# rsokolovskii/fl_scaling_sc_ldpc

Measured on AMD Instinct MI355X. Metric: MC codeword trials/sec, (4,8) SC-LDPC L=50 N=1000 eps=0.48 full BP, higher is better.
Workload: dtype u32

## Files before the change

fl_scaling_sc_ldpc_amd/csrc/sampler_v2.hip:

```cpp
#include "sampler_common.h"
#include "philox.h"

namespace {

using scldpc_dev::channel_erased;
using scldpc_dev::channel_tail;
using scldpc_dev::channel_undope;
using scldpc_dev::clear_hist_words;
using scldpc_dev::load_hist_words;
using scldpc_dev::store_hist_words;
using scldpc_dev::philox4x32_10;
using scldpc_dev::philox_prefix;
using scldpc_dev::philox_tail;
using scldpc_dev::philox_uniform;
using scldpc_dev::PhiloxPrefix;
using scldpc_dev::PhiloxUniform;
using scldpc_dev::wave_inclusive_scan;

constexpr int kThreads = scldpc::kSamplerThreads;
constexpr int kWaves = kThreads / 64;
using scldpc::kMaxDoped;
using scldpc::kWorkCap;

__device__ __forceinline__ uint32_t lds_add_rtn(uint32_t *p, uint32_t v)
{
    const uint32_t addr = (uint32_t)(uintptr_t)(__attribute__((address_space(3))) uint32_t *)p;
    uint32_t old;
    asm volatile("ds_add_rtn_u32 %0, %1, %2\n\ts_waitcnt lgkmcnt(0)" : "=v"(old) : "v"(addr), "v"(v) : "memory");
    return old;
}

struct S2Args {
    int L, cns_pos, vns_pos, n, S, D, nb, nw;
    int ntrials;
    int force_exact;
    int ndoped;
    int doped[kMaxDoped];
    uint32_t seed_lo, seed_hi;
    unsigned long long trial0;
    uint32_t thresh;
    int off_gpk, off_fix, off_stage, off_wsum;
    uint16_t *vn_adj16;
    uint16_t *cn_adj16;
    uint32_t *chan;
};

template <int ROWS, int CNMODE>
struct V2Layout {
    static constexpr int nb = ROWS * kThreads;
    static constexpr int off_gpk = nb, off_fix = off_gpk + nb, off_stage = off_fix + nb / 2;
    static constexpr int off_wsum = off_stage + (CNMODE != 0 ? nb / 2 : 0);
};

template <int KMAX, int ROWS, int CNMODE, bool PERSIST = false>
__global__ __launch_bounds__(kThreads, KMAX == 1 ? 8 : 4) __attribute__((amdgpu_num_sgpr(72))) void sample_philox_v2_kernel(const S2Args a)
{
    constexpr int DV = 4, DC_SHIFT = 3, E = 4 * KMAX;
    constexpr int LG = ROWS == 1 ? 10 : ROWS == 2 ? 11 : ROWS == 4 ? 12 : 13;
    constexpr int KSHIFT = 32 - LG - 2;
    constexpr bool INCL = KMAX == 1;
    static_assert(ROWS * kThreads == (1 << LG) && (INCL ? ROWS <= 4 : ROWS == 8), "ROWS is 1, 2, 4 (KMAX 1) or 8 (KMAX 2)");
    extern __shared__ uint32_t lds[];
    using Lay = V2Layout<ROWS, CNMODE>;
    const int off_gpk = INCL ? Lay::off_gpk : a.off_gpk, off_fix = INCL ? Lay::off_fix : a.off_fix;
    const int off_stage = INCL ? Lay::off_stage : a.off_stage, off_wsum = INCL ? Lay::off_wsum : a.off_wsum;
    uint32_t *hist = lds;
    uint32_t *gpk = lds + off_gpk;
    uint16_t *fix = reinterpret_cast<uint16_t *>(lds + off_fix);
    uint16_t *stage = reinterpret_cast<uint16_t *>(lds + off_stage);
    uint32_t *wsum = lds + off_wsum;
    uint32_t *wl = wsum + 32;

    const int tid = threadIdx.x, lane = tid & 63, wave = __builtin_amdgcn_readfirstlane(tid >> 6);
    const int S = a.S, nb = INCL ? ROWS * kThreads : a.nb;
    const int ncalls = S >> 2;
    bool own[KMAX];
#pragma unroll
    for (int k = 0; k < KMAX; k++) own[k] = tid + k * kThreads < ncalls;
    auto sock = [&](int e) { return (uint32_t)((tid + (e >> 2) * kThreads) * 4 + (e & 3)); };
    auto stage_entry = [&](int p, uint32_t sck) -> uint16_t {
        const int u = (int)(sck & 3u), t = (int)(sck >> 2);
        if ((unsigned)(p - u) >= (unsigned)a.L) return (uint16_t)0xFFFFu;
        return CNMODE == 1 ? (uint16_t)((p - u) * a.vns_pos + t) : (uint16_t)sck;
    };

    STAMP_DECL
    for (int b = tid; b < nb; b += kThreads) hist[b] = 0;
    if (tid == 0) { wsum[kWaves] = 0; wsum[kWaves + 1] = 0; }
    __syncthreads();
    auto sample_trial = [&](const int tr) {
    const unsigned long long trial = a.trial0 + (unsigned long long)tr;
    const uint32_t t_lo = (uint32_t)trial, t_hi = (uint32_t)(trial >> 32);
    uint32_t rowP[KMAX], rowQ[KMAX], rowR[KMAX];
#pragma unroll
    for (int k = 0; k < KMAX; k++) rowP[k] = rowQ[k] = rowR[k] = 0;
    PhiloxPrefix pre[KMAX];
#pragma unroll
    for (int k = 0; k < KMAX; k++) pre[k] = philox_prefix((uint32_t)(tid + k * kThreads), t_lo, t_hi, a.seed_lo, a.seed_hi);
    uint32_t nxt[E];
    {
        const PhiloxUniform un = philox_uniform(0u, t_lo, a.seed_lo, a.seed_hi);
#pragma unroll
        for (int k = 0; k < KMAX; k++) {
            uint32_t r[4] = {0, 0, 0, 0};
            if (own[k]) philox_tail(pre[k], un, a.seed_lo, a.seed_hi, r);
#pragma unroll
            for (int u = 0; u < 4; u++) nxt[4 * k + u] = r[u];
        }
    }
    for (int p = 0; p < a.D; p++) {
        STAMP(0);
        uint32_t key[E], slot[E], crowded = 0;
        auto word_of = [](uint32_t k) { return (k >> KSHIFT) & ~3u; };
        auto nib_of = [](uint32_t k) { return (k >> (KSHIFT - 2)) & 12u; };
#pragma unroll
        for (int e = 0; e < E; e++) {
            key[e] = nxt[e];
            const uint32_t sh = nib_of(key[e]);
            uint32_t *w = reinterpret_cast<uint32_t *>(reinterpret_cast<char *>(hist) + word_of(key[e]));
            slot[e] = (atomicAdd(w, (own[e >> 2] ? 1u : 0u) << sh) >> sh) & 0xFu;
            if constexpr (!INCL) crowded = max(crowded, slot[e]);
        }
        if (!INCL && crowded >= 15u) wsum[kWaves + 1] = 1u;
        __syncthreads();
        STAMP(1);

        const bool ranked = scldpc_dev::scan_hist<ROWS, INCL>(hist, wsum, tid, lane, wave, S);
        STAMP(2);

        if (ranked) {
            uint32_t rk[E], g0a[E], g1a[E];
            bool st[E], sx[E];
            if constexpr (INCL) {
                uint32_t h[E];
#pragma unroll
                for (int e = 0; e < E; e++) h[e] = *reinterpret_cast<const uint32_t *>(reinterpret_cast<const char *>(hist) + word_of(key[e]));
#pragma unroll
                for (int e = 0; e < E; e++) {
                    const uint32_t t = h[e] >> nib_of(key[e]), pre = h[e] >> 20;
                    g0a[e] = pre + (t & 0xFu);
                    g1a[e] = pre + ((t >> 4) & 0xFu);
                    rk[e] = g0a[e] + slot[e];
                    sx[e] = ((g0a[e] ^ (g1a[e] - 1u)) >> DC_SHIFT) != 0u;
                    st[e] = own[e >> 2] && sx[e];
                }
            } else {
                scldpc_dev::bucket_ranges_excl<KSHIFT>(hist, key, [&](int e) { return own[e >> 2]; }, g0a, g1a);
#pragma unroll
                for (int e = 0; e < E; e++) {
                    rk[e] = g0a[e] + slot[e];
                    st[e] = own[e >> 2] && ((g1a[e] - 1u) >> DC_SHIFT) != (g0a[e] >> DC_SHIFT);
                }
            }
            if constexpr (INCL) {
                const unsigned long long ownv = __builtin_amdgcn_ballot_w64(own[0]);
                unsigned long long vote[E];
                int total = 0;
#pragma unroll
                for (int e = 0; e < E; e++) { vote[e] = __builtin_amdgcn_ballot_w64(sx[e]) & ownv; total += __builtin_popcountll(vote[e]); }
                if (total != 0) {
                    uint32_t ln, got = 0;
                    asm volatile("v_and_b32 %0, 63, %1" : "=v"(ln) : "v"(tid));
                    if (ln == 0u) got = lds_add_rtn(&wsum[kWaves], (uint32_t)total);
                    int base = __builtin_amdgcn_readfirstlane((int)got);
                    if (base + total <= kWorkCap) {
                        static_assert((Lay::off_wsum + 32) % 2 == 0, "the worklist starts on a word pair");
                        uint2 *wl2 = reinterpret_cast<uint2 *>(lds);
                        base += (Lay::off_wsum + 32) / 2;
#pragma unroll
                        for (int e = 0; e < E; e++) {
                            if (st[e]) {
                                const uint32_t w = __builtin_amdgcn_mbcnt_hi((uint32_t)(vote[e] >> 32),
                                                                             __builtin_amdgcn_mbcnt_lo((uint32_t)vote[e], (uint32_t)base));
                                const uint32_t pk = (key[e] << LG) | sock(e);
                                gpk[rk[e]] = pk;
                                uint32_t *ent = reinterpret_cast<uint32_t *>(wl2 + w);
                                ent[0] = g0a[e] | (g1a[e] << 16);
                                ent[1] = pk;
                            }
                            base += __builtin_popcountll(vote[e]);
                        }
                    }
                }
            } else {
                uint32_t smask = 0;
#pragma unroll
                for (int e = 0; e < E; e++) smask |= (st[e] ? 1u : 0u) << e;
                while (smask) {
                    const uint32_t e = (uint32_t)__ffs((int)smask) - 1u;
                    smask &= smask - 1u;
                    uint32_t ky = key[0], r0 = rk[0], g0 = g0a[0], g1 = g1a[0];
#pragma unroll
                    for (int f = 1; f < E; f++)
                        if (e == (uint32_t)f) { ky = key[f]; r0 = rk[f]; g0 = g0a[f]; g1 = g1a[f]; }
                    const uint32_t pk = (ky << LG) | (uint32_t)((tid + (int)(e >> 2) * kThreads) * 4 + (int)(e & 3u));
                    gpk[r0] = pk;
                    const int w = atomicAdd(reinterpret_cast<int *>(&wsum[kWaves]), 1);
                    if (w < kWorkCap) { wl[2 * w] = g0 | (g1 << 16); wl[2 * w + 1] = pk; }
                }
            }
#pragma unroll
            for (int k = 0; k < KMAX; k++) {
                if (!own[k]) continue;
                uint2 v;
                v.x = (rk[4 * k] >> DC_SHIFT) | ((rk[4 * k + 1] >> DC_SHIFT) << 16);
                v.y = (rk[4 * k + 2] >> DC_SHIFT) | ((rk[4 * k + 3] >> DC_SHIFT) << 16);
                reinterpret_cast<uint2 *>(fix)[tid + k * kThreads] = v;
            }
            if constexpr (CNMODE != 0) {
#pragma unroll
                for (int k = 0; k < KMAX; k++) {
                    if (!own[k]) continue;
#pragma unroll
                    for (int u = 0; u < 4; u++) stage[rk[4 * k + u]] = stage_entry(p, sock(4 * k + u));
                }
            }
        }
        __syncthreads();
        STAMP(3);

        {
            clear_hist_words<ROWS>(hist, tid);
            int nwork = (int)wsum[kWaves];
            const bool exact = !ranked || nwork > kWorkCap || a.force_exact == p || a.force_exact == -2;
            if (exact) {
                asm volatile("; ledger: cold");
                nwork = 0;
#pragma unroll
                for (int e = 0; e < E; e++) if (own[e >> 2]) gpk[sock(e)] = key[e];
                __syncthreads();
                uint32_t xr[E];
#pragma unroll
                for (int e = 0; e < E; e++) xr[e] = 0;
                for (int s2 = 0; s2 < S; s2++) {
                    const uint32_t k2 = gpk[s2];
#pragma unroll
                    for (int e = 0; e < E; e++) xr[e] += (k2 < key[e]) || (k2 == key[e] && (uint32_t)s2 < sock(e));
                }
#pragma unroll
                for (int k = 0; k < KMAX; k++) {
                    if (!own[k]) continue;
                    uint2 v;
                    v.x = (xr[4 * k] >> DC_SHIFT) | ((xr[4 * k + 1] >> DC_SHIFT) << 16);
                    v.y = (xr[4 * k + 2] >> DC_SHIFT) | ((xr[4 * k + 3] >> DC_SHIFT) << 16);
                    reinterpret_cast<uint2 *>(fix)[tid + k * kThreads] = v;
                    if constexpr (CNMODE != 0) {
#pragma unroll
                        for (int u = 0; u < 4; u++) stage[xr[4 * k + u]] = stage_entry(p, sock(4 * k + u));
                    }
                }
            }
            scldpc_dev::resolve_worklist<LG, CNMODE != 0>(nwork, tid, wl, gpk, stage, fix, [&](uint32_t sck) { return stage_entry(p, sck); },
                                                          [](uint32_t r) { return r >> DC_SHIFT; });
        }
        if (p + 1 < a.D) {
            uint32_t k_lo = a.seed_lo, k_hi = a.seed_hi;
            uint32_t tl = t_lo;
            asm volatile("" : "+s"(k_lo), "+s"(k_hi), "+s"(tl));
            const PhiloxUniform un = philox_uniform((uint32_t)(p + 1), tl, k_lo, k_hi);
#pragma unroll
            for (int k = 0; k < KMAX; k++) {
                uint32_t r[4] = {0, 0, 0, 0};
                if (own[k]) philox_tail(pre[k], un, k_lo, k_hi, r);
#pragma unroll
                for (int u = 0; u < 4; u++) nxt[4 * k + u] = r[u];
            }
        }
        __syncthreads();
        if (tid == 0) { wsum[kWaves] = 0; wsum[kWaves + 1] = 0; }
        STAMP(4);

        const int qpos = p - (DV - 1);
#pragma unroll
        for (int k = 0; k < KMAX; k++) {
            uint2 c = make_uint2(0u, 0u);
            if (own[k]) c = reinterpret_cast<const uint2 *>(fix)[tid + k * kThreads];
            if (qpos >= 0 && own[k]) {
                const size_t j = (size_t)tr * a.n + (size_t)((uint32_t)qpos * (uint32_t)a.vns_pos + (uint32_t)(tid + k * kThreads));
                uint2 v;
                v.x = rowP[k];
                v.y = (rowR[k] >> 16) | (c.y & 0xFFFF0000u);
                reinterpret_cast<uint2 *>(a.vn_adj16)[j] = v;
            }
            rowP[k] = rowQ[k];
            rowQ[k] = (rowR[k] & 0xFFFFu) | (c.x & 0xFFFF0000u);
            rowR[k] = (c.x & 0xFFFFu) | (c.y << 16);
        }
        if constexpr (CNMODE != 0) {
            uint2 *dst = reinterpret_cast<uint2 *>(a.cn_adj16) + ((size_t)tr * a.D + p) * (size_t)(S >> 2);
            const uint2 *src = reinterpret_cast<const uint2 *>(stage);
            for (int w = tid; w < (S >> 2); w += kThreads) dst[w] = src[w];
        }
        STAMP(5);
    }

    uint32_t *chan = a.chan + (size_t)tr * a.nw;
    const PhiloxUniform chun = philox_uniform(0x80000000u, t_lo, a.seed_lo, a.seed_hi);
    for (int w = tid; w < a.nw; w += kThreads) {
        uint32_t word = 0;
#pragma unroll
        for (int c = 0; c < 8; c++) {
            uint32_t r[4];
            philox_tail(philox_prefix((uint32_t)(w * 8 + c), t_lo, t_hi, a.seed_lo, a.seed_hi), chun, a.seed_lo, a.seed_hi, r);
#pragma unroll
            for (int u = 0; u < 4; u++) word |= channel_erased(r[u], a.thresh) << (c * 4 + u);
        }
        const int j0 = w * 32;
        word = channel_tail(word, j0, a.n);
        for (int d = 0; d < a.ndoped; d++) word = channel_undope(word, j0, a.doped[d], a.vns_pos);
        chan[w] = word;
    }
    STAMP(6);
    };
    if constexpr (PERSIST) {
        for (int tr = blockIdx.x; tr < a.ntrials; tr += gridDim.x) {
            sample_trial(tr);
            __syncthreads();
        }
    } else {
        sample_trial((int)blockIdx.x);
    }
    STAMP_FLUSH();
}


__device__ __forceinline__ uint32_t wl_entry_vn(const S2Args &a, int p, uint32_t sck)
{
    return (uint32_t)((p - (int)(sck & 3u)) * a.vns_pos + (int)(sck >> 2));
}

template <int LG, int CNMODE>
__global__ __launch_bounds__(kThreads, 8) __attribute__((amdgpu_num_sgpr(72))) void sample_philox_v3_kernel(const S2Args a)
{
    constexpr int DV = 4, DC_SHIFT = 3, E = 4;
    constexpr int NB = 1 << LG, ROWS = NB / kThreads;
    constexpr int KSHIFT = 32 - LG - 2;
    constexpr uint32_t LOWMASK = (1u << KSHIFT) - 1u;
    constexpr int SBITS = LG;
    static_assert(ROWS == 1 || ROWS == 2 || ROWS == 4, "one Philox call per thread: at most 4096 sockets per position");
    extern __shared__ uint32_t lds[];
    uint32_t *hist0 = lds;
    uint32_t *gpk = lds + a.off_gpk;
    uint16_t *fix = reinterpret_cast<uint16_t *>(lds + a.off_fix);
    uint16_t *stage = reinterpret_cast<uint16_t *>(lds + a.off_stage);
    uint32_t *wsum = lds + a.off_wsum;
    uint32_t *wl = wsum + 32;

    const int tid = threadIdx.x, lane = tid & 63, wave = tid >> 6;
    const int S = a.S;
    const bool own = tid < (S >> 2);
    const unsigned long long trial = a.trial0 + blockIdx.x;
    const uint32_t t_lo = (uint32_t)trial, t_hi = (uint32_t)(trial >> 32);
    const int tr = blockIdx.x;

    STAMP_DECL
    for (int b = tid; b < 2 * NB; b += kThreads) hist0[b] = 0;
    if (tid < 32) wsum[tid] = 0;
    __syncthreads();

    uint32_t rowP = 0, rowQ = 0, rowR = 0;
    uint32_t key[E] = {0, 0, 0, 0}, slot[E] = {0, 0, 0, 0};
    uint32_t ent0 = CNMODE == 1 ? (uint32_t)tid : (uint32_t)(4 * tid);
    uint32_t vV = (uint32_t)a.vns_pos;
    asm volatile("" : "+v"(vV));

    for (int p = 0; p <= a.D; p++) {
        uint32_t *hc = hist0 + (p & 1) * NB, *hp = hist0 + ((p & 1) ^ 1) * NB;
        const bool live = p < a.D;
        STAMP(0);
        if (p > 0) {
            int nwork = (int)wsum[16];
            const bool exact = wsum[18 + ((p - 1) & 1)] != 0u || nwork > kWorkCap || a.force_exact == p - 1 || a.force_exact == -2;
            if (exact) {
                uint32_t k2[4] = {0, 0, 0, 0};
                uint32_t f_lo = a.seed_lo, f_hi = a.seed_hi;
                asm volatile("" : "+s"(f_lo), "+s"(f_hi));
                if (own) philox4x32_10((uint32_t)tid, (uint32_t)(p - 1), t_lo, t_hi, f_lo, f_hi, k2);
                if (own) { gpk[4 * tid] = k2[0]; gpk[4 * tid + 1] = k2[1]; gpk[4 * tid + 2] = k2[2]; gpk[4 * tid + 3] = k2[3]; }
                __syncthreads();
                uint32_t xr[4] = {0, 0, 0, 0};
                for (int s2 = 0; s2 < S; s2++) {
                    const uint32_t kk = gpk[s2];
#pragma unroll
                    for (int u = 0; u < 4; u++) xr[u] += (kk < k2[u]) || (kk == k2[u] && s2 < 4 * tid + u);
                }
                if (own) {
                    uint2 v;
                    v.x = (xr[0] >> DC_SHIFT) | ((xr[1] >> DC_SHIFT) << 16);
                    v.y = (xr[2] >> DC_SHIFT) | ((xr[3] >> DC_SHIFT) << 16);
                    reinterpret_cast<uint2 *>(fix)[tid] = v;
                    if constexpr (CNMODE != 0) {
#pragma unroll
                        for (int u = 0; u < 4; u++) {
                            const int pu = p - 1 - u;
                            stage[xr[u]] = (unsigned)pu < (unsigned)a.L ? (uint16_t)(CNMODE == 1 ? pu * a.vns_pos + tid : 4 * tid + u) : (uint16_t)0xFFFFu;
                        }
                    }
                }
                nwork = 0;
            }
            for (int w = tid; w < nwork; w += kThreads) {
                const uint32_t ea = wl[2 * w], pk = wl[2 * w + 1];
                const uint32_t g0 = ea & 0xFFFFu, cnt = (ea >> 16) & 0xFu, sl = (ea >> 20) & 0xFu;
                uint32_t r = g0;
                for (uint32_t m = 0; m < cnt; m++)
                    if (m != sl) r += gpk[g0 + m] < pk;
                const uint32_t sck = pk & ((1u << SBITS) - 1u);
                if constexpr (CNMODE != 0) stage[r] = (uint16_t)(ea >> 24 ? 0xFFFFu : (CNMODE == 1 ? wl_entry_vn(a, p - 1, sck) : sck));
                fix[sck] = (uint16_t)(r >> DC_SHIFT);
            }
            {
                clear_hist_words<ROWS>(hp, tid);
            }
        }
        STAMP(1);
        if (live) {
            {
                uint32_t k_lo = a.seed_lo, k_hi = a.seed_hi;
                asm volatile("" : "+s"(k_lo), "+s"(k_hi));
                uint32_t r[4] = {0, 0, 0, 0};
                if (own) philox4x32_10((uint32_t)tid, (uint32_t)p, t_lo, t_hi, k_lo, k_hi, r);
#pragma unroll
                for (int u = 0; u < 4; u++) key[u] = r[u];
            }
            uint32_t crowded = 0;
#pragma unroll
            for (int e = 0; e < E; e++) {
                const uint32_t boff = (key[e] >> KSHIFT) & ~3u, sh = (key[e] >> (KSHIFT - 2)) & 12u;
                const uint32_t old = atomicAdd(reinterpret_cast<uint32_t *>(reinterpret_cast<char *>(hc) + boff), (own ? 16u : 0u) << sh);
                slot[e] = (old >> (sh + 4u)) & 0xFu;
                crowded |= slot[e] + 1u;
            }
            if (crowded & 16u) wsum[18 + (p & 1)] = 1u;
        }
        STAMP(2);
        __syncthreads();
        STAMP(3);
        if (tid == 0) { wsum[16] = 0; wsum[18 + ((p & 1) ^ 1)] = 0; }
        if (live) {
            uint32_t x[ROWS], tot = 0, over = 0;
            load_hist_words<ROWS>(hc, tid, x);
            uint32_t v[ROWS];
#pragma unroll
            for (int r = 0; r < ROWS; r++) {
                const uint32_t y = x[r] * 0x1111u;
                const uint32_t sb = (x[r] & 0x0F0F0u) + ((x[r] >> 4) & 0x0F0F0u);
                v[r] = ((sb + (sb >> 8)) >> 4) & 0xFFu;
                over |= v[r];
                x[r] = y & 0xFFFF0u;
                tot += v[r];
            }
            if (over & ~15u) wsum[18 + (p & 1)] = 1u;
            const uint32_t inc = wave_inclusive_scan(tot);
            uint32_t pre = inc - tot;
#pragma unroll
            for (int r = 0; r < ROWS; r++) { x[r] |= pre << 20; pre += v[r]; }
            store_hist_words<ROWS>(hc, tid, x);
            if (lane == 63) wsum[wave] = inc;
        }
        if (p > 0) {
            const int pp = p - 1, qpos = pp - (DV - 1);
            uint2 c = make_uint2(0u, 0u);
            if (own) c = reinterpret_cast<const uint2 *>(fix)[tid];
            if (qpos >= 0 && own) {
                const size_t j = (size_t)tr * a.n + (size_t)qpos * a.vns_pos + (size_t)tid;
                uint2 vv;
                vv.x = rowP;
                vv.y = (rowR >> 16) | (c.y & 0xFFFF0000u);
                reinterpret_cast<uint2 *>(a.vn_adj16)[j] = vv;
            }
            rowP = rowQ;
            rowQ = (rowR & 0xFFFFu) | (c.x & 0xFFFF0000u);
            rowR = (c.x & 0xFFFFu) | (c.y << 16);
            if constexpr (CNMODE != 0) {
                uint2 *dst = reinterpret_cast<uint2 *>(a.cn_adj16) + ((size_t)tr * a.D + pp) * (size_t)(S >> 2);
                const uint2 *src = reinterpret_cast<const uint2 *>(stage);
                if (own) dst[tid] = src[tid];
            }
        }
        STAMP(4);
        __syncthreads();
        STAMP(5);
        if (live && wsum[18 + (p & 1)] == 0u) {
            const uint32_t wt = lane < kWaves ? wsum[lane] : 0u;
            uint32_t wi = wt;
            wi += (uint32_t)__builtin_amdgcn_update_dpp(0, (int)wi, 0x111, 0xF, 0xF, false);
            wi += (uint32_t)__builtin_amdgcn_update_dpp(0, (int)wi, 0x112, 0xF, 0xF, false);
            wi += (uint32_t)__builtin_amdgcn_update_dpp(0, (int)wi, 0x114, 0xF, 0xF, false);
            wi += (uint32_t)__builtin_amdgcn_update_dpp(0, (int)wi, 0x118, 0xF, 0xF, false);
            const uint32_t wex = wi - wt;
            uint32_t h[E], wb[E], rk[E], g0a[E], cnta[E];
#pragma unroll
            for (int e = 0; e < E; e++) h[e] = *reinterpret_cast<const uint32_t *>(reinterpret_cast<const char *>(hc) + ((key[e] >> KSHIFT) & ~3u));
#pragma unroll
            for (int e = 0; e < E; e++) wb[e] = (uint32_t)__builtin_amdgcn_ds_bpermute((int)((key[e] >> 26) & 0x3Cu), (int)wex);
            bool st[E];
            bool anyst = false;
#pragma unroll
            for (int e = 0; e < E; e++) {
                const uint32_t t1 = h[e] >> ((key[e] >> (KSHIFT - 2)) & 12u);
                const uint32_t excl = t1 & 15u, incl = (t1 >> 4) & 15u;
                g0a[e] = (h[e] >> 20) + wb[e] + excl;
                cnta[e] = incl - excl;
                rk[e] = g0a[e] + slot[e];
                st[e] = own && ((g0a[e] ^ (g0a[e] + cnta[e] - 1u)) >> DC_SHIFT) != 0u;
                anyst = anyst || st[e];
            }
            if (own) {
                uint2 vv;
                vv.x = (rk[0] >> DC_SHIFT) | ((rk[1] >> DC_SHIFT) << 16);
                vv.y = (rk[2] >> DC_SHIFT) | ((rk[3] >> DC_SHIFT) << 16);
                reinterpret_cast<uint2 *>(fix)[tid] = vv;
            }
            const bool edge = p < DV - 1 || p >= a.L;
            if constexpr (CNMODE != 0) {
                if (own) {
                    uint32_t ent[E];
                    ent[0] = ent0;
#pragma unroll
                    for (int u = 1; u < 4; u++) ent[u] = CNMODE == 1 ? ent[u - 1] - vV : ent[u - 1] + 1u;
                    if (!edge) {
#pragma unroll
                        for (int u = 0; u < 4; u++) stage[rk[u]] = (uint16_t)ent[u];
                    } else {
#pragma unroll
                        for (int u = 0; u < 4; u++) stage[rk[u]] = (unsigned)(p - u) < (unsigned)a.L ? (uint16_t)ent[u] : (uint16_t)0xFFFFu;
                    }
                }
            }
            if (__builtin_amdgcn_ballot_w64(anyst)) {
                unsigned long long vote[E];
                int total = 0;
#pragma unroll
                for (int e = 0; e < E; e++) { vote[e] = __builtin_amdgcn_ballot_w64(st[e]); total += __builtin_popcountll(vote[e]); }
                int base = 0;
                if (lane == 0) base = atomicAdd(reinterpret_cast<int *>(&wsum[16]), total);
                base = __builtin_amdgcn_readfirstlane(base);
#pragma unroll
                for (int e = 0; e < E; e++) {
                    if (st[e]) {
                        const int w = base + (int)__builtin_amdgcn_mbcnt_hi((uint32_t)(vote[e] >> 32), __builtin_amdgcn_mbcnt_lo((uint32_t)vote[e], 0u));
                        const uint32_t pk = ((key[e] & LOWMASK) << SBITS) | (uint32_t)(4 * tid + e);
                        gpk[g0a[e] + slot[e]] = pk;
                        const uint32_t none = CNMODE != 0 && edge && !((unsigned)(p - e) < (unsigned)a.L) ? 1u : 0u;
                        if (w < kWorkCap) { wl[2 * w] = g0a[e] | (cnta[e] << 16) | (slot[e] << 20) | (none << 24); wl[2 * w + 1] = pk; }
                    }
                    base += __builtin_popcountll(vote[e]);
                }
            }
        }
        if constexpr (CNMODE == 1) ent0 += vV;
        STAMP(6);
        __syncthreads();
        STAMP(7);
    }

    uint32_t *chan = a.chan + (size_t)tr * a.nw;
    for (int w = tid; w < a.nw; w += kThreads) {
        uint32_t word = 0;
        uint32_t c_lo = a.seed_lo, c_hi = a.seed_hi;
        asm volatile("" : "+s"(c_lo), "+s"(c_hi));
#pragma unroll
        for (int c = 0; c < 8; c++) {
            uint32_t r[4];
            philox4x32_10((uint32_t)(w * 8 + c), 0x80000000u, t_lo, t_hi, c_lo, c_hi, r);
#pragma unroll
            for (int u = 0; u < 4; u++) word |= channel_erased(r[u], a.thresh) << (c * 4 + u);
        }
        const int j0 = w * 32;
        word = channel_tail(word, j0, a.n);
        for (int d = 0; d < a.ndoped; d++) word = channel_undope(word, j0, a.doped[d], a.vns_pos);
        chan[w] = word;
    }
    STAMP(8);
    STAMP_FLUSH();
}

int launch_v2(const char *who, int cnmode, const scldpc_code_params *p, uint64_t seed, uint64_t trial0, int32_t ntrials,
              double eps, int32_t ndoped, const int32_t *doped_positions, uint16_t *d_vn_adj16, uint16_t *d_table,
              uint32_t *d_chan_bits, void *stream)
{
    S2Args a{};
    if (int rc = scldpc::check_sample_call(who, p, ntrials < 0 || (ntrials > 0 && (!d_vn_adj16 || !d_chan_bits)), ntrials, eps,
                                           ndoped, doped_positions, &a.ndoped, a.doped)) return rc;
    if (ntrials == 0) return SCLDPC_OK;
    if (!d_table) cnmode = 0;

    a.L = p->L; a.cns_pos = p->cns_pos; a.vns_pos = p->vns_pos;
    a.n = scldpc::n_of(p); a.S = p->cns_pos * p->dc; a.D = p->L + p->dv - 1; a.nw = scldpc::nw_of(p);
    a.seed_lo = (uint32_t)seed; a.seed_hi = (uint32_t)(seed >> 32);
    a.trial0 = trial0;
    a.thresh = scldpc::erasure_threshold(eps);
    const char *gen_env = getenv("SCLDPC_SAMPLER_GEN");
    const bool one_call = a.S <= 4 * kThreads;
    const bool v3 = one_call && gen_env && atoi(gen_env) == 3;
    int lg;
    size_t lds_bytes;
    if (int rc = scldpc::v2_lds_layout(who, a.S, v3 ? 2 : 1, one_call && !v3, cnmode != 0, &a, &lg, &lds_bytes)) return rc;
    a.vn_adj16 = d_vn_adj16; a.cn_adj16 = d_table; a.chan = d_chan_bits;
    a.ntrials = ntrials;

    using Kern = void (*)(const S2Args);
    static const Kern table[4][3] = {
        {sample_philox_v2_kernel<1, 1, 0>, sample_philox_v2_kernel<1, 1, 1>, sample_philox_v2_kernel<1, 1, 2>},
        {sample_philox_v2_kernel<1, 2, 0>, sample_philox_v2_kernel<1, 2, 1>, sample_philox_v2_kernel<1, 2, 2>},
        {sample_philox_v2_kernel<1, 4, 0>, sample_philox_v2_kernel<1, 4, 1>, sample_philox_v2_kernel<1, 4, 2>},
        {sample_philox_v2_kernel<2, 8, 0>, sample_philox_v2_kernel<2, 8, 1>, sample_philox_v2_kernel<2, 8, 2>},
    };
    const int rows = a.nb / kThreads;
    static const Kern table3[3][3] = {
        {sample_philox_v3_kernel<10, 0>, sample_philox_v3_kernel<10, 1>, sample_philox_v3_kernel<10, 2>},
        {sample_philox_v3_kernel<11, 0>, sample_philox_v3_kernel<11, 1>, sample_philox_v3_kernel<11, 2>},
        {sample_philox_v3_kernel<12, 0>, sample_philox_v3_kernel<12, 1>, sample_philox_v3_kernel<12, 2>},
    };
    const int grid = v3 ? ntrials : scldpc::debug_grid("SAMPLER", ntrials);
    Kern kern = v3 ? table3[lg - 10][cnmode] : table[rows == 1 ? 0 : rows == 2 ? 1 : rows == 4 ? 2 : 3][cnmode];
    if (grid < ntrials && rows == 4 && cnmode == 1) kern = sample_philox_v2_kernel<1, 4, 1, true>;
    else if (grid < ntrials) return scldpc::set_error(SCLDPC_ERR_BAD_ARG, "SCLDPC_DEBUG_GRID_SAMPLER: only the <1,4,1> kernel has a persistent form");
    if (int rc_ = scldpc::allow_max_lds(reinterpret_cast<const void *>(kern))) return rc_;
    hipLaunchKernelGGL(kern, dim3(grid), dim3(kThreads), lds_bytes, static_cast<hipStream_t>(stream), a);
    SCLDPC_HIP_CHECK(hipGetLastError());
    return SCLDPC_OK;
}

bool v2_shape(const scldpc_code_params *p)
{
    if (scldpc::check_params(p)) return false;
    const int S = p->cns_pos * p->dc;
    return p->dv == 4 && p->dc == 8 && (S & 3) == 0 && S <= 8192 && p->vns_pos * p->dv == S;
}

}

extern "C" int scldpc_sample_philox_cn16_supported(const scldpc_code_params *p)
{
    return v2_shape(p) && scldpc::n_of(p) < 65535;
}

extern "C" int scldpc_sample_philox_sock16_supported(const scldpc_code_params *p)
{
    return v2_shape(p);
}

extern "C" int scldpc_sample_philox_device_cn16(const scldpc_code_params *p, uint64_t seed, uint64_t trial0,
                                                int32_t ntrials, double eps, int32_t ndoped,
                                                const int32_t *doped_positions, uint16_t *d_vn_adj16,
                                                uint16_t *d_cn_adj16, uint32_t *d_chan_bits, void *stream)
{
    const char *who = "scldpc_sample_philox_device_cn16";
    if (int rc = scldpc::check_params(p)) return rc;
    if (!scldpc_sample_philox_cn16_supported(p))
        return scldpc::set_error(SCLDPC_ERR_TOO_LARGE, "%s: takes dv = 4, dc = 8, at most 8192 sockets per position and "
                                 "fewer than 65535 VNs (got dv=%d dc=%d cns_pos=%d n=%d)", who, p->dv, p->dc, p->cns_pos,
                                 scldpc::n_of(p));
    return launch_v2(who, 1, p, seed, trial0, ntrials, eps, ndoped, doped_positions, d_vn_adj16, d_cn_adj16, d_chan_bits,
                     stream);
}

extern "C" int scldpc_sample_philox_device_sock16(const scldpc_code_params *p, uint64_t seed, uint64_t trial0,
                                                  int32_t ntrials, double eps, int32_t ndoped,
                                                  const int32_t *doped_positions, uint16_t *d_vn_adj16,
                                                  uint16_t *d_cn_sock16, uint32_t *d_chan_bits, void *stream)
{
    const char *who = "scldpc_sample_philox_device_sock16";
    if (int rc = scldpc::check_params(p)) return rc;
    if (!scldpc_sample_philox_sock16_supported(p))
        return scldpc::set_error(SCLDPC_ERR_TOO_LARGE, "%s: takes dv = 4, dc = 8 and at most 8192 sockets per position "
                                 "(got dv=%d dc=%d cns_pos=%d)", who, p->dv, p->dc, p->cns_pos);
    return launch_v2(who, 2, p, seed, trial0, ntrials, eps, ndoped, doped_positions, d_vn_adj16, d_cn_sock16, d_chan_bits,
                     stream);
}
```

Measured before the change: 1.248 million.

## Specialise sampler position loop for full waves and interior positions

The per-position body becomes a generic lambda instantiated with compile-time flags. Full waves skip the per-element ownership checks and ballot masks, and interior positions skip the boundary checks on stage entries, writing them incrementally. The per-position Philox uniforms are precomputed once into LDS, at the cost of extra LDS per trial and a larger code footprint from the duplicated instantiations.

```diff
diff --git a/fl_scaling_sc_ldpc_amd/csrc/sampler_v2.hip b/fl_scaling_sc_ldpc_amd/csrc/sampler_v2.hip
--- a/fl_scaling_sc_ldpc_amd/csrc/sampler_v2.hip
+++ b/fl_scaling_sc_ldpc_amd/csrc/sampler_v2.hip
@@ -1,7 +1,10 @@
 #include "sampler_common.h"
 #include "philox.h"
+#include <type_traits>
 
 namespace {
+
+constexpr bool kOwnForm = true, kInteriorForm = true, kLdsUniform = true;
 
 using scldpc_dev::channel_erased;
 using scldpc_dev::channel_tail;
@@ -59,6 +62,8 @@
     constexpr int LG = ROWS == 1 ? 10 : ROWS == 2 ? 11 : ROWS == 4 ? 12 : 13;
     constexpr int KSHIFT = 32 - LG - 2;
     constexpr bool INCL = KMAX == 1;
+    constexpr bool FORMS = INCL && !PERSIST;
+    constexpr bool OWN_FORM = FORMS && kOwnForm, INTERIOR_FORM = FORMS && kInteriorForm, LDS_UNIFORM = FORMS && kLdsUniform;
     static_assert(ROWS * kThreads == (1 << LG) && (INCL ? ROWS <= 4 : ROWS == 8), "ROWS is 1, 2, 4 (KMAX 1) or 8 (KMAX 2)");
     extern __shared__ uint32_t lds[];
     using Lay = V2Layout<ROWS, CNMODE>;
@@ -70,6 +75,7 @@
     uint16_t *stage = reinterpret_cast<uint16_t *>(lds + off_stage);
     uint32_t *wsum = lds + off_wsum;
     uint32_t *wl = wsum + 32;
+    uint2 *uni = reinterpret_cast<uint2 *>(wl + 2 * kWorkCap);
 
     const int tid = threadIdx.x, lane = tid & 63, wave = __builtin_amdgcn_readfirstlane(tid >> 6);
     const int S = a.S, nb = INCL ? ROWS * kThreads : a.nb;
@@ -97,6 +103,12 @@
     PhiloxPrefix pre[KMAX];
 #pragma unroll
     for (int k = 0; k < KMAX; k++) pre[k] = philox_prefix((uint32_t)(tid + k * kThreads), t_lo, t_hi, a.seed_lo, a.seed_hi);
+    if constexpr (LDS_UNIFORM) {
+        for (int q = tid; q < a.D; q += kThreads) {
+            const PhiloxUniform g = philox_uniform((uint32_t)q, t_lo, a.seed_lo, a.seed_hi);
+            uni[q] = make_uint2(g.u, g.v);
+        }
+    }
     uint32_t nxt[E];
     {
         const PhiloxUniform un = philox_uniform(0u, t_lo, a.seed_lo, a.seed_hi);
@@ -108,7 +120,13 @@
             for (int u = 0; u < 4; u++) nxt[4 * k + u] = r[u];
         }
     }
-    for (int p = 0; p < a.D; p++) {
+    auto position = [&](auto own_all, auto interior, const int p, const uint32_t ent0, const uint32_t vV) {
+        constexpr bool OWN = decltype(own_all)::value, INTERIOR = decltype(interior)::value;
+        auto owns = [&](int k) { return OWN || own[k]; };
+        auto entry_of = [&](uint32_t sck) -> uint16_t {
+            if constexpr (INTERIOR) return CNMODE == 1 ? (uint16_t)((p - (int)(sck & 3u)) * a.vns_pos + (int)(sck >> 2)) : (uint16_t)sck;
+            else return stage_entry(p, sck);
+        };
         STAMP(0);
         uint32_t key[E], slot[E], crowded = 0;
         auto word_of = [](uint32_t k) { return (k >> KSHIFT) & ~3u; };
@@ -118,7 +136,7 @@
             key[e] = nxt[e];
             const uint32_t sh = nib_of(key[e]);
             uint32_t *w = reinterpret_cast<uint32_t *>(reinterpret_cast<char *>(hist) + word_of(key[e]));
-            slot[e] = (atomicAdd(w, (own[e >> 2] ? 1u : 0u) << sh) >> sh) & 0xFu;
+            slot[e] = (atomicAdd(w, (owns(e >> 2) ? 1u : 0u) << sh) >> sh) & 0xFu;
             if constexpr (!INCL) crowded = max(crowded, slot[e]);
         }
         if (!INCL && crowded >= 15u) wsum[kWaves + 1] = 1u;
@@ -142,7 +160,7 @@
                     g1a[e] = pre + ((t >> 4) & 0xFu);
                     rk[e] = g0a[e] + slot[e];
                     sx[e] = ((g0a[e] ^ (g1a[e] - 1u)) >> DC_SHIFT) != 0u;
-                    st[e] = own[e >> 2] && sx[e];
+                    st[e] = owns(e >> 2) && sx[e];
                 }
             } else {
                 scldpc_dev::bucket_ranges_excl<KSHIFT>(hist, key, [&](int e) { return own[e >> 2]; }, g0a, g1a);
@@ -153,11 +171,15 @@
                 }
             }
             if constexpr (INCL) {
-                const unsigned long long ownv = __builtin_amdgcn_ballot_w64(own[0]);
+                const unsigned long long ownv = OWN ? ~0ull : __builtin_amdgcn_ballot_w64(own[0]);
                 unsigned long long vote[E];
                 int total = 0;
 #pragma unroll
-                for (int e = 0; e < E; e++) { vote[e] = __builtin_amdgcn_ballot_w64(sx[e]) & ownv; total += __builtin_popcountll(vote[e]); }
+                for (int e = 0; e < E; e++) {
+                    vote[e] = __builtin_amdgcn_ballot_w64(sx[e]);
+                    if constexpr (!OWN) vote[e] &= ownv;
+                    total += __builtin_popcountll(vote[e]);
+                }
                 if (total != 0) {
                     uint32_t ln, got = 0;
                     asm volatile("v_and_b32 %0, 63, %1" : "=v"(ln) : "v"(tid));
@@ -201,18 +223,25 @@
             }
 #pragma unroll
             for (int k = 0; k < KMAX; k++) {
-                if (!own[k]) continue;
+                if (!owns(k)) continue;
                 uint2 v;
                 v.x = (rk[4 * k] >> DC_SHIFT) | ((rk[4 * k + 1] >> DC_SHIFT) << 16);
                 v.y = (rk[4 * k + 2] >> DC_SHIFT) | ((rk[4 * k + 3] >> DC_SHIFT) << 16);
                 reinterpret_cast<uint2 *>(fix)[tid + k * kThreads] = v;
             }
-            if constexpr (CNMODE != 0) {
+            if constexpr (CNMODE == 1 && INTERIOR) {
+                static_assert(KMAX == 1, "the interior form is the one-call sampler's");
+                if (owns(0)) {
+                    uint32_t ent = ent0;
+#pragma unroll
+                    for (int u = 0; u < 4; u++) { stage[rk[u]] = (uint16_t)ent; ent -= vV; }
+                }
+            } else if constexpr (CNMODE != 0) {
 #pragma unroll
                 for (int k = 0; k < KMAX; k++) {
-                    if (!own[k]) continue;
-#pragma unroll
-                    for (int u = 0; u < 4; u++) stage[rk[4 * k + u]] = stage_entry(p, sock(4 * k + u));
+                    if (!owns(k)) continue;
+#pragma unroll
+                    for (int u = 0; u < 4; u++) stage[rk[4 * k + u]] = entry_of(sock(4 * k + u));
                 }
             }
         }
@@ -227,7 +256,7 @@
                 asm volatile("; ledger: cold");
                 nwork = 0;
 #pragma unroll
-                for (int e = 0; e < E; e++) if (own[e >> 2]) gpk[sock(e)] = key[e];
+                for (int e = 0; e < E; e++) if (owns(e >> 2)) gpk[sock(e)] = key[e];
                 __syncthreads();
                 uint32_t xr[E];
 #pragma unroll
@@ -239,29 +268,31 @@
                 }
 #pragma unroll
                 for (int k = 0; k < KMAX; k++) {
-                    if (!own[k]) continue;
+                    if (!owns(k)) continue;
                     uint2 v;
                     v.x = (xr[4 * k] >> DC_SHIFT) | ((xr[4 * k + 1] >> DC_SHIFT) << 16);
                     v.y = (xr[4 * k + 2] >> DC_SHIFT) | ((xr[4 * k + 3] >> DC_SHIFT) << 16);
                     reinterpret_cast<uint2 *>(fix)[tid + k * kThreads] = v;
                     if constexpr (CNMODE != 0) {
 #pragma unroll
-                        for (int u = 0; u < 4; u++) stage[xr[4 * k + u]] = stage_entry(p, sock(4 * k + u));
+                        for (int u = 0; u < 4; u++) stage[xr[4 * k + u]] = entry_of(sock(4 * k + u));
                     }
                 }
             }
-            scldpc_dev::resolve_worklist<LG, CNMODE != 0>(nwork, tid, wl, gpk, stage, fix, [&](uint32_t sck) { return stage_entry(p, sck); },
+            scldpc_dev::resolve_worklist<LG, CNMODE != 0>(nwork, tid, wl, gpk, stage, fix, entry_of,
                                                           [](uint32_t r) { return r >> DC_SHIFT; });
         }
-        if (p + 1 < a.D) {
+        if (INTERIOR || p + 1 < a.D) {
             uint32_t k_lo = a.seed_lo, k_hi = a.seed_hi;
             uint32_t tl = t_lo;
             asm volatile("" : "+s"(k_lo), "+s"(k_hi), "+s"(tl));
-            const PhiloxUniform un = philox_uniform((uint32_t)(p + 1), tl, k_lo, k_hi);
+            PhiloxUniform un;
+            if constexpr (LDS_UNIFORM) { const uint2 g = uni[p + 1]; un.u = g.x; un.v = g.y; }
+            else un = philox_uniform((uint32_t)(p + 1), tl, k_lo, k_hi);
 #pragma unroll
             for (int k = 0; k < KMAX; k++) {
                 uint32_t r[4] = {0, 0, 0, 0};
-                if (own[k]) philox_tail(pre[k], un, k_lo, k_hi, r);
+                if (owns(k)) philox_tail(pre[k], un, k_lo, k_hi, r);
 #pragma unroll
                 for (int u = 0; u < 4; u++) nxt[4 * k + u] = r[u];
             }
@@ -274,8 +305,8 @@
 #pragma unroll
         for (int k = 0; k < KMAX; k++) {
             uint2 c = make_uint2(0u, 0u);
-            if (own[k]) c = reinterpret_cast<const uint2 *>(fix)[tid + k * kThreads];
-            if (qpos >= 0 && own[k]) {
+            if (owns(k)) c = reinterpret_cast<const uint2 *>(fix)[tid + k * kThreads];
+            if ((INTERIOR || qpos >= 0) && owns(k)) {
                 const size_t j = (size_t)tr * a.n + (size_t)((uint32_t)qpos * (uint32_t)a.vns_pos + (uint32_t)(tid + k * kThreads));
                 uint2 v;
                 v.x = rowP[k];
@@ -289,9 +320,31 @@
         if constexpr (CNMODE != 0) {
             uint2 *dst = reinterpret_cast<uint2 *>(a.cn_adj16) + ((size_t)tr * a.D + p) * (size_t)(S >> 2);
             const uint2 *src = reinterpret_cast<const uint2 *>(stage);
-            for (int w = tid; w < (S >> 2); w += kThreads) dst[w] = src[w];
+            if constexpr (OWN) dst[tid] = src[tid];
+            else for (int w = tid; w < (S >> 2); w += kThreads) dst[w] = src[w];
         }
         STAMP(5);
+    };
+    auto positions = [&](auto own_all) {
+        int p = 0;
+        if constexpr (INTERIOR_FORM) {
+#pragma unroll 1
+            for (; p < DV - 1; p++) position(own_all, std::false_type{}, p, 0u, 0u);
+            uint32_t ent0 = (uint32_t)((DV - 1) * a.vns_pos + tid), vV = (uint32_t)a.vns_pos;
+            asm volatile("" : "+v"(vV));
+#pragma unroll 1
+            for (; p < a.L; p++) { position(own_all, std::true_type{}, p, ent0, vV); ent0 += vV; }
+        }
+#pragma unroll 1
+        for (; p < a.D; p++) {
+            position(own_all, std::false_type{}, p, 0u, 0u);
+        }
+    };
+    if constexpr (OWN_FORM) {
+        if ((wave + 1) * 64 <= ncalls) positions(std::true_type{});
+        else positions(std::false_type{});
+    } else {
+        positions(std::false_type{});
     }
 
     uint32_t *chan = a.chan + (size_t)tr * a.nw;
@@ -597,6 +650,11 @@
     int lg;
     size_t lds_bytes;
     if (int rc = scldpc::v2_lds_layout(who, a.S, v3 ? 2 : 1, one_call && !v3, cnmode != 0, &a, &lg, &lds_bytes)) return rc;
+    if (one_call && !v3) {
+        lds_bytes += 8u * (size_t)a.D;
+        if (lds_bytes > (size_t)scldpc::kMaxLdsBytes)
+            return scldpc::set_error(SCLDPC_ERR_TOO_LARGE, "%s: %zu bytes of LDS per trial", who, lds_bytes);
+    }
     a.vn_adj16 = d_vn_adj16; a.cn_adj16 = d_table; a.chan = d_chan_bits;
     a.ntrials = ntrials;
 
```

New measurement: 1.253 million (median of 6 runs). No clear change (+0.4%).
